# ilur98/DLMC-QUANT

Measured on NVIDIA B200. Metric: fakequant_fwd_bwd_hbm_gbps, higher is better.
Workload: dtype f32

## Files before the change

### dlmc_quant_b200/_lib.py

```python
import ctypes as C
import os

_HERE = os.path.dirname(os.path.abspath(__file__))
LIB_PATH = os.path.join(_HERE, "libdlmcq.so")

F32, BF16 = 0, 1
FORM_A1, FORM_AFFINE, FORM_ZP, FORM_SYM = 0, 1, 2, 3
STATS_PER_CHANNEL = 4
DIV_IEEE, DIV_CUDA_EAGER = 0, 1
SWEEP_CANDIDATES = 80
ROOTQ_STATE_FLOATS = 8
QGEMM_I8, QGEMM_E4M3 = 0, 1


class Layout(C.Structure):
    _fields_ = [("outer", C.c_int64), ("channels", C.c_int64), ("inner", C.c_int64), ("dtype", C.c_int32)]


class QParams(C.Structure):
    _fields_ = [("form", C.c_int32), ("lo", C.c_int32), ("hi", C.c_int32), ("g", C.c_float),
                ("scale", C.c_void_p), ("offset", C.c_void_p)]


class GroupItem(C.Structure):
# ... 36 lines not shown
                ("inner", C.c_int64), ("n_bits", C.c_int32), ("is_signed", C.c_int32), ("wpr", C.c_int32),
                ("row_floats", C.c_int32), ("staged", C.c_int32), ("pad", C.c_int32), ("smem_bytes", C.c_int64),
                ("ctas", C.c_int64)]


class BnqDesc(C.Structure):
    _fields_ = [("rows", C.c_int64), ("channels", C.c_int64), ("dtype", C.c_int32), ("flags", C.c_int32),
                ("eps", C.c_float), ("momentum", C.c_float)]


BNQ_TRAINING, BNQ_RELU, BNQ_RESIDUAL = 1, 2, 4


class DlmcqError(RuntimeError):
    pass


_lib = None

_P, _I, _L, _F, _D, _Z = C.c_void_p, C.c_int, C.c_int64, C.c_float, C.c_double, C.c_size_t
_LP, _QP = C.POINTER(Layout), C.POINTER(QParams)

SIGNATURES = {
    "dlmcq_version": (_I, []),
    "dlmcq_selftest_fastdiv": (_I, [C.c_uint64, _I, _I, _I, _P, _P]),
    "dlmcq_status_string": (C.c_char_p, [_I]),
    "dlmcq_last_cuda_error": (C.c_char_p, []),
    "dlmcq_workspace_bytes": (_Z, [_LP]),
    "dlmcq_fq_forward": (_I, [_P, _P, _P, _LP, _QP, _P]),
    "dlmcq_fq_backward": (_I, [_P, _P, _P, _P, _P, _LP, _QP, _P, _Z, _P]),
    "dlmcq_fq_partials_floats": (_Z, []),
    "dlmcq_fq_backward_partials": (_I, [_P, _P, _P, _LP, _QP, _P, _P]),
    "dlmcq_fq_finalize_many": (_I, [_P, _I, _P]),
    "dlmcq_dequantize": (_I, [_P, _P, _LP, _P, _P, _P]),
    "dlmcq_ste_value": (_I, [_P, _P, _L, _I, _I, _P]),
    "dlmcq_grad_scale_value": (_I, [_P, _P, _L, _F, _P]),
    "dlmcq_export_codes": (_I, [_P, _P, _LP, _QP, _I, _P]),
    "dlmcq_import_codes": (_I, [_P, _P, _LP, _QP, _I, _P]),
    "dlmcq_adaround_forward": (_I, [_P, _P, _P, _LP, _P, _I, _I, _I, _P]),
    "dlmcq_adaround_backward": (_I, [_P, _P, _P, _P, _P, _LP, _P, _I, _I, _P, _Z, _P]),
    "dlmcq_adaround_init_alpha": (_I, [_P, _P, _LP, _P, _P]),
    "dlmcq_rootq_act_prepare": (_I, [_P, _P, _D, _D, _I, _I, _I, _P, _P]),
    "dlmcq_rootq_act_forward": (_I, [_P, _P, _L, _I, _P, _P]),
    "dlmcq_rootq_act_backward": (_I, [_P, _P, _P, _P, _L, _I, _P, _P, _Z, _P]),
    "dlmcq_rootq_wt_prepare": (_I, [_P, _P, _P, _P, _P, _D, _D, _I, _I, _I, _P, _P]),
    "dlmcq_rootq_wt_forward": (_I, [_P, _P, _L, _I, _P, _P]),
    "dlmcq_rootq_wt_backward": (_I, [_P, _P, _P, _P, _L, _I, _P, _P, _Z, _P]),
    "dlmcq_rootq_prepare_many": (_I, [_P, _I, _P]),
    "dlmcq_rootq_wt_forward_grouped": (_I, [_P, _P, _I, _L, _I, _P]),
    "dlmcq_rootq_wt_backward_grouped": (_I, [_P, _P, _I, _L, _I, _P, _P]),
    "dlmcq_rootq_act_forward_grouped": (_I, [_P, _P, _I, _L, _I, _P]),
    "dlmcq_rootq_act_backward_grouped": (_I, [_P, _P, _I, _L, _I, _P, _P]),
    "dlmcq_obs_stats": (_I, [_P, _P, _LP, _I, _P, _Z, _P]),
    "dlmcq_obs_minmax_finalize": (_I, [_P, _P, _P, _L, _I, _I, _I, _P]),
    "dlmcq_obs_minmax_finalize_mode": (_I, [_P, _P, _P, _L, _I, _I, _I, _I, _P]),
    "dlmcq_obs_absmean_finalize": (_I, [_P, _P, _L, _D, _D, _D, _I, _P]),
    "dlmcq_obs_kth_state_bytes": (_Z, []),
    "dlmcq_obs_kth_begin": (_I, [_P, _L, _L, _P]),
    "dlmcq_obs_kth_hist": (_I, [_P, _L, _I, _I, _I, _P, _P]),
    "dlmcq_obs_kth_select": (_I, [_I, _P, _P]),
    "dlmcq_obs_kth_values": (_I, [_P, _P, _P]),
    "dlmcq_obs_kth_fast_workspace_bytes": (_Z, [_L]),
    "dlmcq_obs_kth_fast": (_I, [_P, _L, _I, _I, _L, _L, _P, _P, _P, _Z, _P]),
    "dlmcq_obs_kth_auto": (_I, [_P, _L, _I, _I, _L, _L, _P, _P, _P, _P, _Z, _P]),
    "dlmcq_obs_sweep_tensor_sse": (_I, [_P, _L, _I, _P, _I, _I, _P, _P, _Z, _P]),
    "dlmcq_obs_sweep_tensor_finalize": (_I, [_P, _P, _D, _I, _I, _P, _P, _P, _P]),
# ... 50 lines not shown
```

### dlmc_quant_b200/csrc/fq_kernels.cu

```cuda
#include "fq_rows.cuh"

namespace dlmcq {

constexpr int kUnroll = 4;

template <int FORM, typename T, int U = kUnroll, int MINB = 4, bool TILED = false>
__global__ void __launch_bounds__(kThreads, MINB)
fq_fwd_flat(const T* __restrict__ x, T* __restrict__ y, T* __restrict__ codes, int64_t n,
            const float* __restrict__ scale, const float* __restrict__ offset, float g, float lo, float hi) {
  using V = Vec<T>;
  using raw = typename V::raw;
  pdl_wait();
  pdl_trigger();
  const ChanParams p = make_params<FORM>(scale, offset, 0, g, lo, hi);
  const int64_t nvec = n / V::N;
  const int64_t stride = static_cast<int64_t>(gridDim.x) * blockDim.x;
  int64_t i = static_cast<int64_t>(blockIdx.x) * blockDim.x + threadIdx.x;
  const raw* xv = reinterpret_cast<const raw*>(x);
  raw* yv = reinterpret_cast<raw*>(y);
  raw* cv = reinterpret_cast<raw*>(codes);

  auto body = [&](const raw& r, int64_t idx) {
    float f[V::N], fy[V::N], fc[V::N];
    V::unpack(r, f);
    fq_vec<FORM, V::N>(f, p, lo, hi, fc, fy);
    if (y) st_stream(yv + idx, V::pack(fy));
    if (codes) st_stream(cv + idx, V::pack(fc));
  };
  if (TILED) {
    const int64_t tile_vecs = static_cast<int64_t>(U) * blockDim.x;
    const int64_t ntiles = nvec / tile_vecs;
    for (int64_t t = blockIdx.x; t < ntiles; t += gridDim.x) {
      const int64_t b = t * tile_vecs + threadIdx.x;
      raw r[U];
#pragma unroll
      for (int k = 0; k < U; ++k) r[k] = ld_stream(xv + b + k * blockDim.x);
#pragma unroll
      for (int k = 0; k < U; ++k) body(r[k], b + k * blockDim.x);
    }
    for (int64_t j = ntiles * tile_vecs + i; j < nvec; j += stride) body(ld_stream(xv + j), j);
  } else {
    for (; i + (U - 1) * stride < nvec; i += U * stride) {
      raw r[U];
#pragma unroll
      for (int k = 0; k < U; ++k) r[k] = ld_stream(xv + i + k * stride);
#pragma unroll
      for (int k = 0; k < U; ++k) body(r[k], i + k * stride);
    }
    for (; i < nvec; i += stride) body(ld_stream(xv + i), i);
  }
  if (blockIdx.x == 0) {
    const int64_t t = nvec * V::N + threadIdx.x;
    if (t < n) {
      float c, v;
      fq_elem<FORM>(to_f32<T>(x[t]), p, lo, hi, c, v);
      if (y) y[t] = from_f32<T>(v);
      if (codes) codes[t] = from_f32<T>(c);
    }
  }
}

template <int FORM, typename T>
__global__ void __launch_bounds__(kThreads)
fq_fwd_flat_unaligned(const T* __restrict__ x, T* __restrict__ y, T* __restrict__ codes, int64_t n,
                      const float* __restrict__ scale, const float* __restrict__ offset, float g, float lo, float hi) {
// ... 6 lines not shown
    if (codes) codes[i] = from_f32<T>(c);
  }
}

template <int FORM>
__device__ __forceinline__ void finalize_flat(float* partials, int nblocks, float g, float* dscale, float* doffset,
                                              float* smem) {
  double s = 0.0, o = 0.0;
  for (int b = threadIdx.x; b < nblocks; b += blockDim.x) {
    s += static_cast<double>(partials[2 * b]);
    o += static_cast<double>(partials[2 * b + 1]);
  }
  s = warp_sum(s);
  o = warp_sum(o);
  double* sm = reinterpret_cast<double*>(smem);
  const int lane = threadIdx.x & 31, warp = threadIdx.x >> 5, nwarp = blockDim.x >> 5;
  __syncthreads();
  if (lane == 0) { sm[warp] = s; sm[32 + warp] = o; }
  __syncthreads();
  if (threadIdx.x == 0) {
    double ts = 0.0, to = 0.0;
    for (int w = 0; w < nwarp; ++w) { ts += sm[w]; to += sm[32 + w]; }
    float r = static_cast<float>(ts);
    if (FORM == DLMCQ_FORM_AFFINE || FORM == DLMCQ_FORM_A1) r = r * g;
    dscale[0] = r;
    if (doffset) doffset[0] = static_cast<float>(to);
  }
}

template <int FORM, typename T, bool VECTOR, bool WANT_OFF, bool DEFER>
__global__ void __launch_bounds__(kThreads, 4)
fq_bwd_flat(const T* __restrict__ x, const T* __restrict__ dy, T* __restrict__ dx, int64_t n,
            const float* __restrict__ scale, const float* __restrict__ offset, float g, float lo, float hi,
            float* __restrict__ dscale, float* __restrict__ doffset, void* ws) {
  using V = Vec<T>;
  using raw = typename V::raw;
  __shared__ __align__(16) float smem[128];
  pdl_wait();
  pdl_trigger();
  const ChanParams p = make_params<FORM>(scale, offset, 0, g, lo, hi);
  float acc[2] = {0.f, 0.f};
  const int64_t stride = static_cast<int64_t>(gridDim.x) * blockDim.x;
  int64_t i = static_cast<int64_t>(blockIdx.x) * blockDim.x + threadIdx.x;
  if (VECTOR) {
    const int64_t nvec = n / V::N;
    const raw* xv = reinterpret_cast<const raw*>(x);
    const raw* gv = reinterpret_cast<const raw*>(dy);
    raw* ov = reinterpret_cast<raw*>(dx);
    auto body = [&](const raw& rx, const raw& rg, int64_t idx) {
      float fx[V::N], fg[V::N], fo[V::N];
      V::unpack(rx, fx);
      V::unpack(rg, fg);
      fq_vec_bwd<FORM, WANT_OFF, V::N>(fx, fg, p, lo, hi, fo, acc[0], acc[1]);
      st_stream(ov + idx, V::pack(fo));
    };
    const int64_t tile_vecs = static_cast<int64_t>(kUnroll) * blockDim.x;
    const int64_t ntiles = nvec / tile_vecs;
    for (int64_t t = blockIdx.x; t < ntiles; t += gridDim.x) {
      const int64_t b = t * tile_vecs + threadIdx.x;
      raw rx[kUnroll], rg[kUnroll];
#pragma unroll
      for (int k = 0; k < kUnroll; ++k) {
        rx[k] = ld_stream(xv + b + k * blockDim.x);
        rg[k] = ld_stream(gv + b + k * blockDim.x);
      }
#pragma unroll
      for (int k = 0; k < kUnroll; ++k) body(rx[k], rg[k], b + k * blockDim.x);
    }
    for (int64_t j = ntiles * tile_vecs + i; j < nvec; j += stride) body(ld_stream(xv + j), ld_stream(gv + j), j);
    if (blockIdx.x == 0) {
      const int64_t t = nvec * V::N + threadIdx.x;
      if (t < n) dx[t] = from_f32<T>(fq_elem_bwd<FORM, WANT_OFF>(to_f32<T>(x[t]), to_f32<T>(dy[t]), p, lo, hi, acc[0], acc[1]));
    }
  } else {
    for (; i < n; i += stride)
      dx[i] = from_f32<T>(fq_elem_bwd<FORM, WANT_OFF>(to_f32<T>(x[i]), to_f32<T>(dy[i]), p, lo, hi, acc[0], acc[1]));
  }
  block_sum<2>(acc, smem);
  if (DEFER) {
    float* out = static_cast<float*>(ws);
    if (threadIdx.x == 0) {
      if (blockIdx.x == 0) {
        out[0] = __int_as_float(static_cast<int>(gridDim.x));
        out[1] = (FORM == DLMCQ_FORM_AFFINE || FORM == DLMCQ_FORM_A1) ? g : 1.f;
      }
      out[2 + 2 * blockIdx.x] = acc[0];
      out[3 + 2 * blockIdx.x] = acc[1];
    }
    return;
  }
  float* partials = ws_partials(ws);
// ... 336 lines not shown
  }
}

__global__ void __launch_bounds__(128)
tiled_chan_finalize(const float* __restrict__ part, TileGeom gm, int64_t outer, float gmul, float* __restrict__ dscale) {
  __shared__ double sh[4];
  const int64_t ch = blockIdx.x;
  double s = 0.0;
  for (int64_t b = threadIdx.x; b < outer; b += blockDim.x) {
    const int64_t row = b * gm.channels + ch;
    const int64_t t0 = (row * gm.vpr) / kTileVecs, t1 = ((row + 1) * gm.vpr - 1) / kTileVecs;
    for (int64_t t = t0; t <= t1; ++t) {
      const int64_t row_first = (t * kTileVecs) / gm.vpr;
      s += static_cast<double>(part[t * kTileRows + (row - row_first)]);
    }
  }
  s = warp_sum(s);
  if ((threadIdx.x & 31) == 0) sh[threadIdx.x >> 5] = s;
  __syncthreads();
  if (threadIdx.x == 0) dscale[ch] = static_cast<float>((sh[0] + sh[1]) + (sh[2] + sh[3])) * gmul;
}

static inline int check_layout(const dlmcq_layout* l) {
  if (!l || l->outer < 1 || l->channels < 1 || l->inner < 0) return DLMCQ_EINVAL;
  if (l->dtype != DLMCQ_F32 && l->dtype != DLMCQ_BF16) return DLMCQ_EINVAL;
  return DLMCQ_OK;
}
static inline size_t elem_size(int dtype) { return dtype == DLMCQ_F32 ? 4 : 2; }
static inline bool elem_aligned(const void* p, int dtype) {
  return p == nullptr || (reinterpret_cast<uintptr_t>(p) % elem_size(dtype)) == 0;
}
static inline RowGeom make_geom(const dlmcq_layout* l) { return make_geom(l->outer, l->channels, l->inner); }

template <int FORM, typename T>
static int launch_fwd(const void* x, void* y, void* codes, const dlmcq_layout* l, const dlmcq_qparams* qp,
                      cudaStream_t st) {
  const int64_t n = l->outer * l->channels * l->inner;
  if (n == 0) return DLMCQ_OK;
  const float lo = static_cast<float>(qp->lo), hi = static_cast<float>(qp->hi);
  if (l->channels == 1) {
    if (aligned16(x) && aligned16(y) && aligned16(codes)) {
      const int64_t tiles = (n / Vec<T>::N + kThreads * kUnroll - 1) / (kThreads * kUnroll);
      auto kern = fq_fwd_flat<FORM, T, kUnroll, 4, true>;
      const int bps = 1024;
      cudaError_t e = launch_pdl(kern, dim3(stream_grid(tiles, bps)), dim3(kThreads), 0, st,
                                 static_cast<const T*>(x), static_cast<T*>(y), static_cast<T*>(codes), n, qp->scale,
                                 qp->offset, qp->g, lo, hi);
      if (e != cudaSuccess) return set_cuda_error(e);
    } else {
      const int64_t tiles = (n + kThreads - 1) / kThreads;
      fq_fwd_flat_unaligned<FORM, T><<<stream_grid(tiles, 8), kThreads, 0, st>>>(
          static_cast<const T*>(x), static_cast<T*>(y), static_cast<T*>(codes), n, qp->scale, qp->offset, qp->g, lo, hi);
    }
  } else if (tiled_ok<T>(l, x, y, codes)) {
    const TileGeom tg = make_tile_geom<T>(l);
    const int64_t tiles = (tg.nvec + kTileVecs - 1) / kTileVecs;
    if (tiles > 0x7fffffffLL) return DLMCQ_EUNSUPPORTED;
    fq_tiled_chan_kernel<FORM, T, false><<<static_cast<unsigned>(tiles), kThreads, 0, st>>>(
        static_cast<const T*>(x), nullptr, static_cast<T*>(y), static_cast<T*>(codes), tg, qp->scale, qp->offset,
        qp->g, lo, hi, nullptr);
  } else if (slab_ok<T>(l->outer, l->channels, l->inner, x, y, codes, nullptr)) {
    const SlabGeom sg = make_slab<T>(l->outer, l->channels, l->inner);
    fq_slab_kernel<FORM, T><<<static_cast<unsigned>(sg.groups) * sg.chunks, kThreads, 0, st>>>(
        static_cast<const T*>(x), static_cast<T*>(y), static_cast<T*>(codes), sg, qp->scale, qp->offset, qp->g, lo, hi);
  } else if (cmaj_ok(l->outer, l->channels, l->inner)) {
    const bool vec = cmaj_vec_ok<T>(l->inner, x, y, codes, nullptr);
    const CmajGeom cg = make_cmaj(l->outer, l->channels, l->inner, vec ? Vec<T>::N : 1);
    const int64_t blocks = (cg.channels * cg.chunks + kRowWarps - 1) / kRowWarps;
    if (blocks > 0x7fffffffLL) return DLMCQ_EUNSUPPORTED;
    auto kern = vec ? fq_cmaj_kernel<FORM, T, false, Vec<T>::N> : fq_cmaj_kernel<FORM, T, false, 1>;
    kern<<<static_cast<unsigned>(blocks), kRowWarps * 32, 0, st>>>(
        static_cast<const T*>(x), nullptr, static_cast<T*>(y), static_cast<T*>(codes), cg, qp->scale, qp->offset,
        qp->g, lo, hi, nullptr, nullptr, 0);
  } else {
    const RowGeom gm = make_geom(l);
    const int64_t items = gm.rows * gm.segs;
    const int64_t blocks = (items + kRowWarps - 1) / kRowWarps;
    if (blocks > 0x7fffffffLL) return DLMCQ_EUNSUPPORTED;
    fq_fwd_rows<FORM, T><<<static_cast<unsigned>(blocks), kRowWarps * 32, 0, st>>>(
        static_cast<const T*>(x), static_cast<T*>(y), static_cast<T*>(codes), gm, qp->scale, qp->offset, qp->g, lo, hi);
  }
  DLMCQ_LAUNCH_CHECK();
  return DLMCQ_OK;
}

template <int FORM, typename T>
static int launch_bwd(const void* x, const void* dy, void* dx, float* dscale, float* doffset, const dlmcq_layout* l,
                      const dlmcq_qparams* qp, void* ws, size_t ws_bytes, cudaStream_t st, bool defer = false) {
  const int64_t n = l->outer * l->channels * l->inner;
  const float lo = static_cast<float>(qp->lo), hi = static_cast<float>(qp->hi);
  if (!defer && ws_bytes < dlmcq_workspace_bytes(l)) return DLMCQ_EWORKSPACE;
  if (defer && l->channels != 1) return DLMCQ_EUNSUPPORTED;
  if (l->channels == 1) {
    const bool vec = aligned16(x) && aligned16(dy) && aligned16(dx);
    const int64_t per = vec ? Vec<T>::N : 1;
    int64_t tiles = (n / per + kThreads * kUnroll - 1) / (kThreads * kUnroll);
    int64_t cap = n < (int64_t(1) << 25) ? 888 : (n < (int64_t(1) << 27) ? 2048 : 4096);
    if (cap > kMaxPartialBlocks) cap = kMaxPartialBlocks;
    const int grid = static_cast<int>(tiles < 1 ? 1 : (tiles < cap ? tiles : cap));
    auto k = vec ? (doffset ? fq_bwd_flat<FORM, T, true, true, false> : fq_bwd_flat<FORM, T, true, false, false>)
                 : (doffset ? fq_bwd_flat<FORM, T, false, true, false> : fq_bwd_flat<FORM, T, false, false, false>);
    if (defer) k = vec ? fq_bwd_flat<FORM, T, true, false, true> : fq_bwd_flat<FORM, T, false, false, true>;
    cudaError_t e = launch_pdl(k, dim3(grid), dim3(kThreads), 0, st, static_cast<const T*>(x),
                               static_cast<const T*>(dy), static_cast<T*>(dx), n, qp->scale, qp->offset, qp->g, lo, hi,
                               dscale, doffset, ws);
    if (e != cudaSuccess) return set_cuda_error(e);
  } else if (doffset == nullptr && n > 0 && tiled_ok<T>(l, x, dy, dx)) {
    const TileGeom tg = make_tile_geom<T>(l);
    const int64_t tiles = (tg.nvec + kTileVecs - 1) / kTileVecs;
    if (tiles > 0x7fffffffLL) return DLMCQ_EUNSUPPORTED;
    fq_tiled_chan_kernel<FORM, T, true><<<static_cast<unsigned>(tiles), kThreads, 0, st>>>(
        static_cast<const T*>(x), static_cast<const T*>(dy), static_cast<T*>(dx), nullptr, tg, qp->scale, qp->offset,
        qp->g, lo, hi, ws_partials(ws));
    DLMCQ_LAUNCH_CHECK();
    const float gmul = (FORM == DLMCQ_FORM_AFFINE || FORM == DLMCQ_FORM_A1) ? qp->g : 1.f;
    tiled_chan_finalize<<<static_cast<unsigned>(l->channels), 128, 0, st>>>(ws_partials(ws), tg, l->outer, gmul, dscale);
  } else if (cmaj_ok(l->outer, l->channels, l->inner) && doffset == nullptr && n > 0) {
    const bool vec = cmaj_vec_ok<T>(l->inner, x, dy, dx, nullptr);
    const CmajGeom cg = make_cmaj(l->outer, l->channels, l->inner, vec ? Vec<T>::N : 1);
    const int64_t blocks = (cg.channels * cg.chunks + kRowWarps - 1) / kRowWarps;
    if (blocks > 0x7fffffffLL) return DLMCQ_EUNSUPPORTED;
    const int direct = cg.chunks == 1 ? 1 : 0;
    auto kern = vec ? fq_cmaj_kernel<FORM, T, true, Vec<T>::N> : fq_cmaj_kernel<FORM, T, true, 1>;
    kern<<<static_cast<unsigned>(blocks), kRowWarps * 32, 0, st>>>(
        static_cast<const T*>(x), static_cast<const T*>(dy), static_cast<T*>(dx), nullptr, cg, qp->scale, qp->offset,
        qp->g, lo, hi, dscale, ws_partials(ws), direct);
    if (!direct) {
      DLMCQ_LAUNCH_CHECK();
      const float gmul = (FORM == DLMCQ_FORM_AFFINE || FORM == DLMCQ_FORM_A1) ? qp->g : 1.f;
      chan_finalize<1><<<static_cast<unsigned>(cg.channels), 128, 0, st>>>(ws_partials(ws), cg.chunks, cg.chunks, 0,
                                                                           gmul, dscale, nullptr);
    }
  } else {
    const RowGeom gm = make_geom(l);
    const int64_t items = gm.rows * gm.segs;
    const int64_t blocks = (items + kRowWarps - 1) / kRowWarps;
    if (blocks > 0x7fffffffLL) return DLMCQ_EUNSUPPORTED;
    const int direct = (l->outer == 1 && gm.segs == 1) ? 1 : 0;
    if (n == 0) return DLMCQ_OK;
// ... 7 lines not shown
          ws_partials(ws), l->outer * gm.segs, gm.segs, gm.channels * gm.segs, gmul, dscale, doffset);
    }
  }
  DLMCQ_LAUNCH_CHECK();
  return DLMCQ_OK;
}

template <typename T>
static int dispatch_fwd(const void* x, void* y, void* codes, const dlmcq_layout* l, const dlmcq_qparams* qp,
                        cudaStream_t st) {
  switch (qp->form) {
    case DLMCQ_FORM_A1: return launch_fwd<DLMCQ_FORM_A1, T>(x, y, codes, l, qp, st);
    case DLMCQ_FORM_AFFINE: return launch_fwd<DLMCQ_FORM_AFFINE, T>(x, y, codes, l, qp, st);
    case DLMCQ_FORM_ZP: return launch_fwd<DLMCQ_FORM_ZP, T>(x, y, codes, l, qp, st);
    case DLMCQ_FORM_SYM: return launch_fwd<DLMCQ_FORM_SYM, T>(x, y, codes, l, qp, st);
  }
  return DLMCQ_EINVAL;
}
template <typename T>
static int dispatch_bwd(const void* x, const void* dy, void* dx, float* ds, float* doff, const dlmcq_layout* l,
                        const dlmcq_qparams* qp, void* ws, size_t wsb, cudaStream_t st, bool defer = false) {
  switch (qp->form) {
    case DLMCQ_FORM_A1: return launch_bwd<DLMCQ_FORM_A1, T>(x, dy, dx, ds, doff, l, qp, ws, wsb, st, defer);
    case DLMCQ_FORM_AFFINE: return launch_bwd<DLMCQ_FORM_AFFINE, T>(x, dy, dx, ds, doff, l, qp, ws, wsb, st, defer);
    case DLMCQ_FORM_ZP: return launch_bwd<DLMCQ_FORM_ZP, T>(x, dy, dx, ds, doff, l, qp, ws, wsb, st, defer);
    case DLMCQ_FORM_SYM: return launch_bwd<DLMCQ_FORM_SYM, T>(x, dy, dx, ds, doff, l, qp, ws, wsb, st, defer);
  }
  return DLMCQ_EINVAL;
}

__global__ void __launch_bounds__(kThreads)
finalize_many_kernel(const dlmcq_finalize_item* __restrict__ items, int n_items) {
  __shared__ double sm[2][kThreads / 32];
  const dlmcq_finalize_item it = items[blockIdx.x];
  const float* p = it.partials;
  const int nblocks = __float_as_int(p[0]);
  const float gmul = p[1];
  double s = 0.0, o = 0.0;
  for (int b = threadIdx.x; b < nblocks; b += blockDim.x) {
    s += static_cast<double>(p[2 + 2 * b]);
    o += static_cast<double>(p[3 + 2 * b]);
  }
  s = warp_sum(s);
  o = warp_sum(o);
  const int lane = threadIdx.x & 31, warp = threadIdx.x >> 5;
  if (lane == 0) { sm[0][warp] = s; sm[1][warp] = o; }
  __syncthreads();
  if (threadIdx.x == 0) {
    double ts = 0.0, to = 0.0;
    for (int w = 0; w < kThreads / 32; ++w) { ts += sm[0][w]; to += sm[1][w]; }
    it.dscale[0] = static_cast<float>(ts) * gmul;
    (void)to;
  }
}

}

using namespace dlmcq;

extern "C" size_t dlmcq_workspace_bytes(const dlmcq_layout* l) {
  size_t bytes = kWsHeaderBytes + static_cast<size_t>(kMaxPartialBlocks) * 96 * sizeof(float);
  if (l && l->outer >= 1 && l->channels >= 1 && l->inner >= 0) {
    const RowGeom gm = make_geom(l->outer, l->channels, l->inner);
    const size_t rows_bytes = static_cast<size_t>(gm.rows * gm.segs) * 4 * sizeof(float);
    if (kWsHeaderBytes + rows_bytes > bytes) bytes = kWsHeaderBytes + rows_bytes;
    const size_t tiles = static_cast<size_t>(l->outer * l->channels * l->inner) / (kTileVecs * 4) + 1;
// ... 33 lines not shown
                                const float* offset, void* stream) {
  if (int e = check_layout(layout)) return e;
  if (!codes || !y || !scale) return DLMCQ_EINVAL;
  const int64_t n = layout->outer * layout->channels * layout->inner;
  if (n == 0) return DLMCQ_OK;
  cudaStream_t st = static_cast<cudaStream_t>(stream);
  const int grid = stream_grid((n + kThreads - 1) / kThreads, 8);
  if (layout->dtype == DLMCQ_F32)
    dequant_kernel<float><<<grid, kThreads, 0, st>>>(static_cast<const float*>(codes), static_cast<float*>(y), n,
                                                     layout->channels, layout->inner, scale, offset);
  else
    dequant_kernel<__nv_bfloat16><<<grid, kThreads, 0, st>>>(static_cast<const __nv_bfloat16*>(codes),
                                                             static_cast<__nv_bfloat16*>(y), n, layout->channels,
                                                             layout->inner, scale, offset);
  DLMCQ_LAUNCH_CHECK();
  return DLMCQ_OK;
}

extern "C" size_t dlmcq_fq_partials_floats(void) { return 2 + 2 * static_cast<size_t>(kMaxPartialBlocks); }

extern "C" int dlmcq_fq_backward_partials(const void* x, const void* dy, void* dx, const dlmcq_layout* layout,
                                          const dlmcq_qparams* qp, float* partials, void* stream) {
  if (int e = check_layout(layout)) return e;
  if (layout->channels != 1) return DLMCQ_EUNSUPPORTED;
  if (!qp || !qp->scale || !partials || !x || !dy || !dx) return DLMCQ_EINVAL;
  if (!elem_aligned(x, layout->dtype) || !elem_aligned(dy, layout->dtype) || !elem_aligned(dx, layout->dtype))
    return DLMCQ_EALIGN;
  cudaStream_t st = static_cast<cudaStream_t>(stream);
  return layout->dtype == DLMCQ_F32
             ? dispatch_bwd<float>(x, dy, dx, nullptr, nullptr, layout, qp, partials, 0, st, true)
             : dispatch_bwd<__nv_bfloat16>(x, dy, dx, nullptr, nullptr, layout, qp, partials, 0, st, true);
}

extern "C" int dlmcq_fq_finalize_many(const dlmcq_finalize_item* items, int n_items, void* stream) {
  if (!items || n_items < 0) return DLMCQ_EINVAL;
  if (n_items == 0) return DLMCQ_OK;
  finalize_many_kernel<<<n_items, kThreads, 0, static_cast<cudaStream_t>(stream)>>>(items, n_items);
  DLMCQ_LAUNCH_CHECK();
  return DLMCQ_OK;
}
```

### dlmc_quant_b200/csrc/grouped_kernels.cu

```cuda
#include "fq_rows.cuh"

namespace dlmcq {

__device__ __forceinline__ int find_item(const int64_t* __restrict__ prefix, int n_items, int64_t unit) {
  int lo = 0, hi = n_items;
  while (hi - lo > 1) {
    const int mid = (lo + hi) >> 1;
    if (__ldg(prefix + mid) <= unit) lo = mid; else hi = mid;
  }
  return lo;
}

template <int FORM>
__device__ __forceinline__ ChanParams item_params(const dlmcq_group_item& it, int64_t ch) {
  return make_params<FORM>(it.scale, it.offset, ch, it.g, static_cast<float>(it.lo), static_cast<float>(it.hi));
}

template <typename T>
__global__ void __launch_bounds__(kRowWarps * 32)
grouped_fwd_kernel(const dlmcq_group_item* __restrict__ items, const int64_t* __restrict__ prefix, int n_items,
                   int64_t total_units) {
  const int lane = threadIdx.x & 31;
  const int64_t unit = static_cast<int64_t>(blockIdx.x) * kRowWarps + (threadIdx.x >> 5);
  if (unit >= total_units) return;
  const int k = find_item(prefix, n_items, unit);
  const dlmcq_group_item it = items[k];
  const int64_t local = unit - __ldg(prefix + k);
  const int64_t segs = (it.inner + DLMCQ_GROUP_SEG - 1) / DLMCQ_GROUP_SEG;
  const int64_t row = local / segs, seg = local - row * segs;
  const int64_t beg = seg * DLMCQ_GROUP_SEG;
  const int64_t len = (it.inner - beg) < DLMCQ_GROUP_SEG ? (it.inner - beg) : DLMCQ_GROUP_SEG;
  const T* xr = static_cast<const T*>(it.x) + row * it.inner + beg;
  T* yr = static_cast<T*>(it.y) + row * it.inner + beg;
  const float lo = static_cast<float>(it.lo), hi = static_cast<float>(it.hi);
  switch (it.form) {
    case DLMCQ_FORM_A1: fwd_row_segment<DLMCQ_FORM_A1, T>(xr, yr, nullptr, len, item_params<DLMCQ_FORM_A1>(it, row), lo, hi, lane); break;
    case DLMCQ_FORM_AFFINE: fwd_row_segment<DLMCQ_FORM_AFFINE, T>(xr, yr, nullptr, len, item_params<DLMCQ_FORM_AFFINE>(it, row), lo, hi, lane); break;
    case DLMCQ_FORM_ZP: fwd_row_segment<DLMCQ_FORM_ZP, T>(xr, yr, nullptr, len, item_params<DLMCQ_FORM_ZP>(it, row), lo, hi, lane); break;
    default: fwd_row_segment<DLMCQ_FORM_SYM, T>(xr, yr, nullptr, len, item_params<DLMCQ_FORM_SYM>(it, row), lo, hi, lane); break;
  }
}

template <typename T>
__global__ void __launch_bounds__(kRowWarps * 32)
grouped_bwd_kernel(const dlmcq_group_item* __restrict__ items, const int64_t* __restrict__ prefix, int n_items,
                   int64_t total_units, float* __restrict__ partials) {
  const int lane = threadIdx.x & 31;
  const int64_t unit = static_cast<int64_t>(blockIdx.x) * kRowWarps + (threadIdx.x >> 5);
  if (unit >= total_units) return;
  const int k = find_item(prefix, n_items, unit);
  const dlmcq_group_item it = items[k];
  const int64_t local = unit - __ldg(prefix + k);
  const int64_t segs = (it.inner + DLMCQ_GROUP_SEG - 1) / DLMCQ_GROUP_SEG;
  const int64_t row = local / segs, seg = local - row * segs;
  const int64_t beg = seg * DLMCQ_GROUP_SEG;
  const int64_t len = (it.inner - beg) < DLMCQ_GROUP_SEG ? (it.inner - beg) : DLMCQ_GROUP_SEG;
  const int64_t base = row * it.inner + beg;
  const T* xr = static_cast<const T*>(it.x) + base;
  const T* gr = static_cast<const T*>(it.dy) + base;
  T* dr = static_cast<T*>(it.y) + base;
  const float lo = static_cast<float>(it.lo), hi = static_cast<float>(it.hi);
  float as = 0.f, ao = 0.f;
  switch (it.form) {
    case DLMCQ_FORM_A1: bwd_row_segment<DLMCQ_FORM_A1, T>(xr, gr, dr, len, item_params<DLMCQ_FORM_A1>(it, row), lo, hi, lane, as, ao); break;
    case DLMCQ_FORM_AFFINE: bwd_row_segment<DLMCQ_FORM_AFFINE, T>(xr, gr, dr, len, item_params<DLMCQ_FORM_AFFINE>(it, row), lo, hi, lane, as, ao); break;
    case DLMCQ_FORM_ZP: bwd_row_segment<DLMCQ_FORM_ZP, T>(xr, gr, dr, len, item_params<DLMCQ_FORM_ZP>(it, row), lo, hi, lane, as, ao); break;
    default: bwd_row_segment<DLMCQ_FORM_SYM, T>(xr, gr, dr, len, item_params<DLMCQ_FORM_SYM>(it, row), lo, hi, lane, as, ao); break;
  }
  if (lane == 0) partials[unit] = as;
}

__global__ void __launch_bounds__(kRowWarps * 32)
grouped_finalize_kernel(const dlmcq_group_item* __restrict__ items, const int64_t* __restrict__ prefix,
                        const int64_t* __restrict__ chan_prefix, int n_items, int64_t total_channels,
                        const float* __restrict__ partials) {
  const int lane = threadIdx.x & 31;
  const int64_t gch = static_cast<int64_t>(blockIdx.x) * kRowWarps + (threadIdx.x >> 5);
  if (gch >= total_channels) return;
  const int k = find_item(chan_prefix, n_items, gch);
  const dlmcq_group_item it = items[k];
  const int64_t ch = gch - __ldg(chan_prefix + k);
  const int64_t segs = (it.inner + DLMCQ_GROUP_SEG - 1) / DLMCQ_GROUP_SEG;
  const float* p = partials + __ldg(prefix + k) + ch * segs;
  double s = 0.0;
  for (int64_t j = lane; j < segs; j += 32) s += static_cast<double>(p[j]);
  s = warp_sum(s);
  if (lane == 0) {
    float r = static_cast<float>(s);
    if (it.form == DLMCQ_FORM_AFFINE || it.form == DLMCQ_FORM_A1) r = r * it.g;
    it.dscale[ch] = r;
  }
}

}

using namespace dlmcq;

extern "C" int dlmcq_fq_forward_grouped(const dlmcq_group_item* items, const int64_t* unit_prefix, int n_items,
                                        int64_t total_units, int dtype, void* stream) {
  if (!items || !unit_prefix || n_items < 1 || total_units < 0) return DLMCQ_EINVAL;
  if (total_units == 0) return DLMCQ_OK;
  const int64_t blocks = (total_units + kRowWarps - 1) / kRowWarps;
  if (blocks > 0x7fffffffLL) return DLMCQ_EUNSUPPORTED;
  cudaStream_t st = static_cast<cudaStream_t>(stream);
  if (dtype == DLMCQ_F32)
    grouped_fwd_kernel<float><<<static_cast<unsigned>(blocks), kRowWarps * 32, 0, st>>>(items, unit_prefix, n_items, total_units);
  else if (dtype == DLMCQ_BF16)
    grouped_fwd_kernel<__nv_bfloat16><<<static_cast<unsigned>(blocks), kRowWarps * 32, 0, st>>>(items, unit_prefix, n_items, total_units);
  else
    return DLMCQ_EINVAL;
  DLMCQ_LAUNCH_CHECK();
  return DLMCQ_OK;
}

extern "C" int dlmcq_fq_backward_grouped(const dlmcq_group_item* items, const int64_t* unit_prefix,
                                         const int64_t* chan_prefix, int n_items, int64_t total_units,
                                         int64_t total_channels, int dtype, float* partials, void* stream) {
  if (!items || !unit_prefix || !chan_prefix || !partials || n_items < 1 || total_units < 0) return DLMCQ_EINVAL;
  if (total_units == 0) return DLMCQ_OK;
  const int64_t blocks = (total_units + kRowWarps - 1) / kRowWarps;
  const int64_t fblocks = (total_channels + kRowWarps - 1) / kRowWarps;
  if (blocks > 0x7fffffffLL || fblocks > 0x7fffffffLL) return DLMCQ_EUNSUPPORTED;
  cudaStream_t st = static_cast<cudaStream_t>(stream);
  if (dtype == DLMCQ_F32)
    grouped_bwd_kernel<float><<<static_cast<unsigned>(blocks), kRowWarps * 32, 0, st>>>(items, unit_prefix, n_items, total_units, partials);
  else if (dtype == DLMCQ_BF16)
    grouped_bwd_kernel<__nv_bfloat16><<<static_cast<unsigned>(blocks), kRowWarps * 32, 0, st>>>(items, unit_prefix, n_items, total_units, partials);
  else
    return DLMCQ_EINVAL;
  DLMCQ_LAUNCH_CHECK();
  grouped_finalize_kernel<<<static_cast<unsigned>(fblocks), kRowWarps * 32, 0, st>>>(items, unit_prefix, chan_prefix, n_items, total_channels, partials);
  DLMCQ_LAUNCH_CHECK();
  return DLMCQ_OK;
}
```

### include/dlmcq.h

```cpp
#ifndef DLMCQ_H_
#define DLMCQ_H_

#include <stddef.h>
#include <stdint.h>

#ifdef __cplusplus
extern "C" {
#endif

#define DLMCQ_VERSION 100

typedef enum {
  DLMCQ_OK = 0,
  DLMCQ_EINVAL = -1,
  DLMCQ_EALIGN = -2,
  DLMCQ_EWORKSPACE = -3,
  DLMCQ_ECUDA = -4,
  DLMCQ_EUNSUPPORTED = -5
} dlmcq_status;

typedef enum { DLMCQ_F32 = 0, DLMCQ_BF16 = 1 } dlmcq_dtype;

typedef enum {
  DLMCQ_FORM_A1 = 0,
// ... 10 lines not shown
} dlmcq_layout;

typedef struct {
  int32_t form;
  int32_t lo, hi;
  float g;
  const float* scale;
  const float* offset;
} dlmcq_qparams;

int dlmcq_version(void);
int dlmcq_selftest_fastdiv(uint64_t seed, int blocks, int per_thread, int narrow,
                           unsigned long long* mismatches_dev, void* stream);
const char* dlmcq_status_string(int status);
const char* dlmcq_last_cuda_error(void);

size_t dlmcq_workspace_bytes(const dlmcq_layout* layout);

int dlmcq_fq_forward(const void* x, void* y, void* codes, const dlmcq_layout* layout,
                     const dlmcq_qparams* qp, void* stream);

int dlmcq_fq_backward(const void* x, const void* dy, void* dx, float* dscale, float* doffset,
                      const dlmcq_layout* layout, const dlmcq_qparams* qp,
                      void* workspace, size_t workspace_bytes, void* stream);

typedef struct {
  const float* partials;
  float* dscale;
} dlmcq_finalize_item;
size_t dlmcq_fq_partials_floats(void);
int dlmcq_fq_backward_partials(const void* x, const void* dy, void* dx, const dlmcq_layout* layout,
                               const dlmcq_qparams* qp, float* partials, void* stream);
int dlmcq_fq_finalize_many(const dlmcq_finalize_item* items, int n_items, void* stream);

int dlmcq_ste_value(const void* x, void* y, int64_t numel, int dtype, int mode, void* stream);
int dlmcq_grad_scale_value(const float* s, float* out, int64_t numel, float g, void* stream);

int dlmcq_dequantize(const void* codes, void* y, const dlmcq_layout* layout,
                     const float* scale, const float* offset, void* stream);

int dlmcq_export_codes(const void* x, void* codes_out, const dlmcq_layout* layout, const dlmcq_qparams* qp,
                       int pack4, void* stream);
int dlmcq_import_codes(const void* codes, void* y, const dlmcq_layout* layout, const dlmcq_qparams* qp,
                       int pack4, void* stream);

int dlmcq_adaround_forward(const void* w, const void* alpha, void* y, const dlmcq_layout* layout,
                           const float* scale, int lo, int hi, int soft, void* stream);
int dlmcq_adaround_backward(const void* w, const void* alpha, const void* dy, void* dalpha,
                            float* dscale, const dlmcq_layout* layout, const float* scale,
                            int lo, int hi, void* workspace, size_t workspace_bytes, void* stream);
int dlmcq_adaround_init_alpha(const void* w, void* alpha, const dlmcq_layout* layout,
                              const float* scale, void* stream);

#define DLMCQ_ROOTQ_STATE_FLOATS 8

int dlmcq_rootq_act_prepare(const float* in_scale, float* run_scale, double momentum, double g,
                            int lo, int hi, int training, float* state, void* stream);
int dlmcq_rootq_act_forward(const void* x, void* y, int64_t numel, int dtype,
                            const float* state, void* stream);
int dlmcq_rootq_act_backward(const void* x, const void* dy, void* dx, float* d_in_scale,
                             int64_t numel, int dtype, const float* state,
                             void* workspace, size_t workspace_bytes, void* stream);
int dlmcq_rootq_wt_prepare(const float* upper, const float* lower, const float* alpha,
                           float* run_upper, float* run_lower, double momentum, double g,
                           int lo, int hi, int training, float* state, void* stream);
int dlmcq_rootq_wt_forward(const void* w, void* y, int64_t numel, int dtype,
// ... 177 lines not shown
```

Measured before the change: 6293.

## Prefetch first tile before PDL wait when captured kernels touch disjoint memory

During CUDA graph capture, each flat fake-quant launch records the byte ranges it reads and writes, and checks them against the previous captured node. When the ranges do not overlap, the kernel loads its first tile and quant params before pdl_wait, so its memory reads overlap the tail of the previous kernel. Finalize and grouped kernels are also moved to PDL launches with wait/trigger. The cost is host-side bookkeeping with a mutex and extra registers for the hoisted tile, and correctness depends on the alias check covering every dependency.

```diff
diff --git a/dlmc_quant_b200/_lib.py b/dlmc_quant_b200/_lib.py
--- a/dlmc_quant_b200/_lib.py
+++ b/dlmc_quant_b200/_lib.py
@@ -92,6 +92,7 @@
     "dlmcq_fq_partials_floats": (_Z, []),
     "dlmcq_fq_backward_partials": (_I, [_P, _P, _P, _LP, _QP, _P, _P]),
     "dlmcq_fq_finalize_many": (_I, [_P, _I, _P]),
+    "dlmcq_capture_overlap_count": (_I, []),
     "dlmcq_dequantize": (_I, [_P, _P, _LP, _P, _P, _P]),
     "dlmcq_ste_value": (_I, [_P, _P, _L, _I, _I, _P]),
     "dlmcq_grad_scale_value": (_I, [_P, _P, _L, _F, _P]),
diff --git a/dlmc_quant_b200/csrc/fq_kernels.cu b/dlmc_quant_b200/csrc/fq_kernels.cu
--- a/dlmc_quant_b200/csrc/fq_kernels.cu
+++ b/dlmc_quant_b200/csrc/fq_kernels.cu
@@ -1,3 +1,5 @@
+#include <mutex>
+
 #include "fq_rows.cuh"
 
 namespace dlmcq {
@@ -7,16 +9,30 @@
 template <int FORM, typename T, int U = kUnroll, int MINB = 4, bool TILED = false>
 __global__ void __launch_bounds__(kThreads, MINB)
 fq_fwd_flat(const T* __restrict__ x, T* __restrict__ y, T* __restrict__ codes, int64_t n,
-            const float* __restrict__ scale, const float* __restrict__ offset, float g, float lo, float hi) {
+            const float* __restrict__ scale, const float* __restrict__ offset, float g, float lo, float hi,
+            int independent) {
   using V = Vec<T>;
   using raw = typename V::raw;
+  const int64_t nvec = n / V::N;
+  const raw* xv = reinterpret_cast<const raw*>(x);
+  const int64_t tile_vecs = static_cast<int64_t>(U) * blockDim.x;
+  const int64_t ntiles = nvec / tile_vecs;
+  ChanParams p;
+  raw r0[U];
+  const bool hoist = TILED && independent && blockIdx.x < ntiles;
+  if (TILED && independent) {
+    p = make_params<FORM>(scale, offset, 0, g, lo, hi);
+    if (hoist) {
+      const int64_t b = static_cast<int64_t>(blockIdx.x) * tile_vecs + threadIdx.x;
+#pragma unroll
+      for (int k = 0; k < U; ++k) r0[k] = ld_stream(xv + b + k * blockDim.x);
+    }
+  }
   pdl_wait();
   pdl_trigger();
-  const ChanParams p = make_params<FORM>(scale, offset, 0, g, lo, hi);
-  const int64_t nvec = n / V::N;
+  if (!(TILED && independent)) p = make_params<FORM>(scale, offset, 0, g, lo, hi);
   const int64_t stride = static_cast<int64_t>(gridDim.x) * blockDim.x;
   int64_t i = static_cast<int64_t>(blockIdx.x) * blockDim.x + threadIdx.x;
-  const raw* xv = reinterpret_cast<const raw*>(x);
   raw* yv = reinterpret_cast<raw*>(y);
   raw* cv = reinterpret_cast<raw*>(codes);
 
@@ -28,9 +44,14 @@
     if (codes) st_stream(cv + idx, V::pack(fc));
   };
   if (TILED) {
-    const int64_t tile_vecs = static_cast<int64_t>(U) * blockDim.x;
-    const int64_t ntiles = nvec / tile_vecs;
-    for (int64_t t = blockIdx.x; t < ntiles; t += gridDim.x) {
+    int64_t t = blockIdx.x;
+    if (hoist) {
+      const int64_t b = t * tile_vecs + threadIdx.x;
+#pragma unroll
+      for (int k = 0; k < U; ++k) body(r0[k], b + k * blockDim.x);
+      t += gridDim.x;
+    }
+    for (; t < ntiles; t += gridDim.x) {
       const int64_t b = t * tile_vecs + threadIdx.x;
       raw r[U];
 #pragma unroll
@@ -103,20 +124,36 @@
 __global__ void __launch_bounds__(kThreads, 4)
 fq_bwd_flat(const T* __restrict__ x, const T* __restrict__ dy, T* __restrict__ dx, int64_t n,
             const float* __restrict__ scale, const float* __restrict__ offset, float g, float lo, float hi,
-            float* __restrict__ dscale, float* __restrict__ doffset, void* ws) {
+            float* __restrict__ dscale, float* __restrict__ doffset, void* ws, int independent) {
   using V = Vec<T>;
   using raw = typename V::raw;
   __shared__ __align__(16) float smem[128];
+  const int64_t nvec = n / V::N;
+  const raw* xv = reinterpret_cast<const raw*>(x);
+  const raw* gv = reinterpret_cast<const raw*>(dy);
+  const int64_t tile_vecs = static_cast<int64_t>(kUnroll) * blockDim.x;
+  const int64_t ntiles = nvec / tile_vecs;
+  ChanParams p;
+  raw rx0[kUnroll], rg0[kUnroll];
+  const bool hoist = VECTOR && independent && blockIdx.x < ntiles;
+  if (VECTOR && independent) {
+    p = make_params<FORM>(scale, offset, 0, g, lo, hi);
+    if (hoist) {
+      const int64_t b = static_cast<int64_t>(blockIdx.x) * tile_vecs + threadIdx.x;
+#pragma unroll
+      for (int k = 0; k < kUnroll; ++k) {
+        rx0[k] = ld_stream(xv + b + k * blockDim.x);
+        rg0[k] = ld_stream(gv + b + k * blockDim.x);
+      }
+    }
+  }
   pdl_wait();
   pdl_trigger();
-  const ChanParams p = make_params<FORM>(scale, offset, 0, g, lo, hi);
+  if (!(VECTOR && independent)) p = make_params<FORM>(scale, offset, 0, g, lo, hi);
   float acc[2] = {0.f, 0.f};
   const int64_t stride = static_cast<int64_t>(gridDim.x) * blockDim.x;
   int64_t i = static_cast<int64_t>(blockIdx.x) * blockDim.x + threadIdx.x;
   if (VECTOR) {
-    const int64_t nvec = n / V::N;
-    const raw* xv = reinterpret_cast<const raw*>(x);
-    const raw* gv = reinterpret_cast<const raw*>(dy);
     raw* ov = reinterpret_cast<raw*>(dx);
     auto body = [&](const raw& rx, const raw& rg, int64_t idx) {
       float fx[V::N], fg[V::N], fo[V::N];
@@ -125,9 +162,14 @@
       fq_vec_bwd<FORM, WANT_OFF, V::N>(fx, fg, p, lo, hi, fo, acc[0], acc[1]);
       st_stream(ov + idx, V::pack(fo));
     };
-    const int64_t tile_vecs = static_cast<int64_t>(kUnroll) * blockDim.x;
-    const int64_t ntiles = nvec / tile_vecs;
-    for (int64_t t = blockIdx.x; t < ntiles; t += gridDim.x) {
+    int64_t t = blockIdx.x;
+    if (hoist) {
+      const int64_t b = t * tile_vecs + threadIdx.x;
+#pragma unroll
+      for (int k = 0; k < kUnroll; ++k) body(rx0[k], rg0[k], b + k * blockDim.x);
+      t += gridDim.x;
+    }
+    for (; t < ntiles; t += gridDim.x) {
       const int64_t b = t * tile_vecs + threadIdx.x;
       raw rx[kUnroll], rg[kUnroll];
 #pragma unroll
@@ -530,6 +572,73 @@
 }
 static inline RowGeom make_geom(const dlmcq_layout* l) { return make_geom(l->outer, l->channels, l->inner); }
 
+struct ByteRange {
+  uintptr_t beg, end;
+};
+struct FlatAccess {
+  ByteRange rd[5], wr[6];
+  int nrd = 0, nwr = 0;
+  void read(const void* p, size_t bytes) {
+    if (p && bytes) rd[nrd++] = {reinterpret_cast<uintptr_t>(p), reinterpret_cast<uintptr_t>(p) + bytes};
+  }
+  void write(const void* p, size_t bytes) {
+    if (p && bytes) wr[nwr++] = {reinterpret_cast<uintptr_t>(p), reinterpret_cast<uintptr_t>(p) + bytes};
+  }
+};
+struct CaptureLast {
+  unsigned long long id;
+  cudaGraphNode_t node;
+  FlatAccess acc;
+};
+constexpr int kCaptureSlots = 16;
+static std::mutex g_capture_mu;
+static CaptureLast g_capture[kCaptureSlots];
+static int g_capture_next = 0;
+static thread_local int g_overlap_count = 0;
+
+static bool capture_tip(cudaStream_t st, unsigned long long* id, cudaGraphNode_t* node) {
+  cudaStreamCaptureStatus status = cudaStreamCaptureStatusNone;
+  const cudaGraphNode_t* deps = nullptr;
+  size_t ndeps = 0;
+  if (cudaStreamGetCaptureInfo(st, &status, id, nullptr, &deps, &ndeps) != cudaSuccess) {
+    (void)cudaGetLastError();
+    return false;
+  }
+  if (status != cudaStreamCaptureStatusActive || ndeps != 1 || deps[0] == nullptr) return false;
+  *node = deps[0];
+  return true;
+}
+
+static int capture_check(cudaStream_t st, const FlatAccess& a) {
+  unsigned long long id = 0;
+  cudaGraphNode_t node = nullptr;
+  if (!pdl_enabled() || !capture_tip(st, &id, &node)) return 0;
+  std::lock_guard<std::mutex> lock(g_capture_mu);
+  for (const CaptureLast& c : g_capture) {
+    if (c.node != node || c.id != id) continue;
+    for (int r = 0; r < a.nrd; ++r)
+      for (int w = 0; w < c.acc.nwr; ++w)
+        if (a.rd[r].beg < c.acc.wr[w].end && c.acc.wr[w].beg < a.rd[r].end) return 0;
+    return 1;
+  }
+  return 0;
+}
+
+static void capture_record(cudaStream_t st, const FlatAccess& a, int independent) {
+  unsigned long long id = 0;
+  cudaGraphNode_t node = nullptr;
+  if (!pdl_enabled() || !capture_tip(st, &id, &node)) return;
+  if (independent) ++g_overlap_count;
+  std::lock_guard<std::mutex> lock(g_capture_mu);
+  CaptureLast* slot = nullptr;
+  for (CaptureLast& c : g_capture)
+    if (c.node != nullptr && c.id == id) slot = &c;
+  if (!slot) slot = &g_capture[g_capture_next++ % kCaptureSlots];
+  slot->id = id;
+  slot->node = node;
+  slot->acc = a;
+}
+
 template <int FORM, typename T>
 static int launch_fwd(const void* x, void* y, void* codes, const dlmcq_layout* l, const dlmcq_qparams* qp,
                       cudaStream_t st) {
@@ -541,10 +650,19 @@
       const int64_t tiles = (n / Vec<T>::N + kThreads * kUnroll - 1) / (kThreads * kUnroll);
       auto kern = fq_fwd_flat<FORM, T, kUnroll, 4, true>;
       const int bps = 1024;
+      const size_t bytes = static_cast<size_t>(n) * sizeof(T);
+      FlatAccess acc;
+      acc.read(x, bytes);
+      acc.read(qp->scale, sizeof(float));
+      acc.read(qp->offset, sizeof(float));
+      acc.write(y, bytes);
+      acc.write(codes, bytes);
+      const int independent = capture_check(st, acc);
       cudaError_t e = launch_pdl(kern, dim3(stream_grid(tiles, bps)), dim3(kThreads), 0, st,
                                  static_cast<const T*>(x), static_cast<T*>(y), static_cast<T*>(codes), n, qp->scale,
-                                 qp->offset, qp->g, lo, hi);
+                                 qp->offset, qp->g, lo, hi, independent);
       if (e != cudaSuccess) return set_cuda_error(e);
+      capture_record(st, acc, independent);
     } else {
       const int64_t tiles = (n + kThreads - 1) / kThreads;
       fq_fwd_flat_unaligned<FORM, T><<<stream_grid(tiles, 8), kThreads, 0, st>>>(
@@ -599,10 +717,25 @@
     auto k = vec ? (doffset ? fq_bwd_flat<FORM, T, true, true, false> : fq_bwd_flat<FORM, T, true, false, false>)
                  : (doffset ? fq_bwd_flat<FORM, T, false, true, false> : fq_bwd_flat<FORM, T, false, false, false>);
     if (defer) k = vec ? fq_bwd_flat<FORM, T, true, false, true> : fq_bwd_flat<FORM, T, false, false, true>;
+    FlatAccess acc;
+    if (vec) {
+      const size_t bytes = static_cast<size_t>(n) * sizeof(T);
+      acc.read(x, bytes);
+      acc.read(dy, bytes);
+      acc.read(qp->scale, sizeof(float));
+      acc.read(qp->offset, sizeof(float));
+      if (!defer) acc.read(ws, ws_bytes);
+      acc.write(dx, bytes);
+      acc.write(dscale, sizeof(float));
+      acc.write(doffset, sizeof(float));
+      acc.write(ws, defer ? (2 + 2 * static_cast<size_t>(grid)) * sizeof(float) : ws_bytes);
+    }
+    const int independent = vec ? capture_check(st, acc) : 0;
     cudaError_t e = launch_pdl(k, dim3(grid), dim3(kThreads), 0, st, static_cast<const T*>(x),
                                static_cast<const T*>(dy), static_cast<T*>(dx), n, qp->scale, qp->offset, qp->g, lo, hi,
-                               dscale, doffset, ws);
+                               dscale, doffset, ws, independent);
     if (e != cudaSuccess) return set_cuda_error(e);
+    if (vec) capture_record(st, acc, independent);
   } else if (doffset == nullptr && n > 0 && tiled_ok<T>(l, x, dy, dx)) {
     const TileGeom tg = make_tile_geom<T>(l);
     const int64_t tiles = (tg.nvec + kTileVecs - 1) / kTileVecs;
@@ -676,6 +809,8 @@
 __global__ void __launch_bounds__(kThreads)
 finalize_many_kernel(const dlmcq_finalize_item* __restrict__ items, int n_items) {
   __shared__ double sm[2][kThreads / 32];
+  pdl_wait();
+  pdl_trigger();
   const dlmcq_finalize_item it = items[blockIdx.x];
   const float* p = it.partials;
   const int nblocks = __float_as_int(p[0]);
@@ -775,10 +910,17 @@
              : dispatch_bwd<__nv_bfloat16>(x, dy, dx, nullptr, nullptr, layout, qp, partials, 0, st, true);
 }
 
+extern "C" int dlmcq_capture_overlap_count(void) {
+  const int n = g_overlap_count;
+  g_overlap_count = 0;
+  return n;
+}
+
 extern "C" int dlmcq_fq_finalize_many(const dlmcq_finalize_item* items, int n_items, void* stream) {
   if (!items || n_items < 0) return DLMCQ_EINVAL;
   if (n_items == 0) return DLMCQ_OK;
-  finalize_many_kernel<<<n_items, kThreads, 0, static_cast<cudaStream_t>(stream)>>>(items, n_items);
-  DLMCQ_LAUNCH_CHECK();
+  cudaError_t e = launch_pdl(finalize_many_kernel, dim3(n_items), dim3(kThreads), 0, static_cast<cudaStream_t>(stream),
+                             items, n_items);
+  if (e != cudaSuccess) return set_cuda_error(e);
   return DLMCQ_OK;
 }
diff --git a/dlmc_quant_b200/csrc/grouped_kernels.cu b/dlmc_quant_b200/csrc/grouped_kernels.cu
--- a/dlmc_quant_b200/csrc/grouped_kernels.cu
+++ b/dlmc_quant_b200/csrc/grouped_kernels.cu
@@ -20,6 +20,8 @@
 __global__ void __launch_bounds__(kRowWarps * 32)
 grouped_fwd_kernel(const dlmcq_group_item* __restrict__ items, const int64_t* __restrict__ prefix, int n_items,
                    int64_t total_units) {
+  pdl_wait();
+  pdl_trigger();
   const int lane = threadIdx.x & 31;
   const int64_t unit = static_cast<int64_t>(blockIdx.x) * kRowWarps + (threadIdx.x >> 5);
   if (unit >= total_units) return;
@@ -45,6 +47,8 @@
 __global__ void __launch_bounds__(kRowWarps * 32)
 grouped_bwd_kernel(const dlmcq_group_item* __restrict__ items, const int64_t* __restrict__ prefix, int n_items,
                    int64_t total_units, float* __restrict__ partials) {
+  pdl_wait();
+  pdl_trigger();
   const int lane = threadIdx.x & 31;
   const int64_t unit = static_cast<int64_t>(blockIdx.x) * kRowWarps + (threadIdx.x >> 5);
   if (unit >= total_units) return;
@@ -74,6 +78,8 @@
 grouped_finalize_kernel(const dlmcq_group_item* __restrict__ items, const int64_t* __restrict__ prefix,
                         const int64_t* __restrict__ chan_prefix, int n_items, int64_t total_channels,
                         const float* __restrict__ partials) {
+  pdl_wait();
+  pdl_trigger();
   const int lane = threadIdx.x & 31;
   const int64_t gch = static_cast<int64_t>(blockIdx.x) * kRowWarps + (threadIdx.x >> 5);
   if (gch >= total_channels) return;
@@ -103,13 +109,11 @@
   const int64_t blocks = (total_units + kRowWarps - 1) / kRowWarps;
   if (blocks > 0x7fffffffLL) return DLMCQ_EUNSUPPORTED;
   cudaStream_t st = static_cast<cudaStream_t>(stream);
-  if (dtype == DLMCQ_F32)
-    grouped_fwd_kernel<float><<<static_cast<unsigned>(blocks), kRowWarps * 32, 0, st>>>(items, unit_prefix, n_items, total_units);
-  else if (dtype == DLMCQ_BF16)
-    grouped_fwd_kernel<__nv_bfloat16><<<static_cast<unsigned>(blocks), kRowWarps * 32, 0, st>>>(items, unit_prefix, n_items, total_units);
-  else
-    return DLMCQ_EINVAL;
-  DLMCQ_LAUNCH_CHECK();
+  if (dtype != DLMCQ_F32 && dtype != DLMCQ_BF16) return DLMCQ_EINVAL;
+  cudaError_t e = launch_pdl(dtype == DLMCQ_F32 ? grouped_fwd_kernel<float> : grouped_fwd_kernel<__nv_bfloat16>,
+                             dim3(static_cast<unsigned>(blocks)), dim3(kRowWarps * 32), 0, st, items, unit_prefix,
+                             n_items, total_units);
+  if (e != cudaSuccess) return set_cuda_error(e);
   return DLMCQ_OK;
 }
 
@@ -122,14 +126,13 @@
   const int64_t fblocks = (total_channels + kRowWarps - 1) / kRowWarps;
   if (blocks > 0x7fffffffLL || fblocks > 0x7fffffffLL) return DLMCQ_EUNSUPPORTED;
   cudaStream_t st = static_cast<cudaStream_t>(stream);
-  if (dtype == DLMCQ_F32)
-    grouped_bwd_kernel<float><<<static_cast<unsigned>(blocks), kRowWarps * 32, 0, st>>>(items, unit_prefix, n_items, total_units, partials);
-  else if (dtype == DLMCQ_BF16)
-    grouped_bwd_kernel<__nv_bfloat16><<<static_cast<unsigned>(blocks), kRowWarps * 32, 0, st>>>(items, unit_prefix, n_items, total_units, partials);
-  else
-    return DLMCQ_EINVAL;
-  DLMCQ_LAUNCH_CHECK();
-  grouped_finalize_kernel<<<static_cast<unsigned>(fblocks), kRowWarps * 32, 0, st>>>(items, unit_prefix, chan_prefix, n_items, total_channels, partials);
-  DLMCQ_LAUNCH_CHECK();
+  if (dtype != DLMCQ_F32 && dtype != DLMCQ_BF16) return DLMCQ_EINVAL;
+  cudaError_t e = launch_pdl(dtype == DLMCQ_F32 ? grouped_bwd_kernel<float> : grouped_bwd_kernel<__nv_bfloat16>,
+                             dim3(static_cast<unsigned>(blocks)), dim3(kRowWarps * 32), 0, st, items, unit_prefix,
+                             n_items, total_units, partials);
+  if (e != cudaSuccess) return set_cuda_error(e);
+  e = launch_pdl(grouped_finalize_kernel, dim3(static_cast<unsigned>(fblocks)), dim3(kRowWarps * 32), 0, st, items,
+                 unit_prefix, chan_prefix, n_items, total_channels, partials);
+  if (e != cudaSuccess) return set_cuda_error(e);
   return DLMCQ_OK;
 }
diff --git a/include/dlmcq.h b/include/dlmcq.h
--- a/include/dlmcq.h
+++ b/include/dlmcq.h
@@ -66,6 +66,8 @@
 int dlmcq_fq_backward_partials(const void* x, const void* dy, void* dx, const dlmcq_layout* layout,
                                const dlmcq_qparams* qp, float* partials, void* stream);
 int dlmcq_fq_finalize_many(const dlmcq_finalize_item* items, int n_items, void* stream);
+
+int dlmcq_capture_overlap_count(void);
 
 int dlmcq_ste_value(const void* x, void* y, int64_t numel, int dtype, int mode, void* stream);
 int dlmcq_grad_scale_value(const float* s, float* out, int64_t numel, float g, void* stream);
diff --git a/profiles/capture_gaps.py b/profiles/capture_gaps.py
--- /dev/null
+++ b/profiles/capture_gaps.py
@@ -0,0 +1,64 @@
+import argparse
+import json
+import os
+import statistics
+import sys
+
+ROOT = os.path.dirname(os.path.dirname(os.path.abspath(__file__)))
+if ROOT not in sys.path:
+    sys.path.insert(0, ROOT)
+
+
+def main():
+    ap = argparse.ArgumentParser()
+    ap.add_argument("--batch", type=int, default=128)
+    ap.add_argument("--steps", type=int, default=3)
+    ap.add_argument("--out", default=None)
+    args = ap.parse_args()
+    import torch
+    from torch.profiler import ProfilerActivity, profile
+
+    import bench
+    wl = bench.Workload(args.batch, torch.device("cuda"), 2333)
+    wl.capture()
+    for _ in range(3):
+        wl.g_fwd.replay(); wl.g_bwd.replay(); wl.g_wt.replay()
+    torch.cuda.synchronize()
+    with profile(activities=[ProfilerActivity.CUDA]) as prof:
+        for _ in range(args.steps):
+            wl.g_fwd.replay(); wl.g_bwd.replay(); wl.g_wt.replay()
+        torch.cuda.synchronize()
+    kernels = sorted((e for e in prof.events() if e.device_type == torch.autograd.DeviceType.CUDA
+                      and e.name not in ("Memcpy", "Memset")), key=lambda e: e.time_range.start)
+    per_step = wl.launches_per_step
+    if len(kernels) < per_step * args.steps:
+        raise SystemExit(f"expected {per_step * args.steps} kernels in the trace, found {len(kernels)}")
+    step = kernels[-per_step:]
+    rows, gaps, adv = [], {"fwd": [], "bwd": [], "other": []}, {"fwd": [], "bwd": [], "other": []}
+    for a, b in zip(step, step[1:]):
+        gap = b.time_range.start - a.time_range.end
+        kind = ("fwd" if "fq_fwd_flat" in a.name and "fq_fwd_flat" in b.name else
+                "bwd" if "fq_bwd_flat" in a.name and "fq_bwd_flat" in b.name else "other")
+        advance = b.time_range.end - a.time_range.end
+        gaps[kind].append(gap)
+        adv[kind].append(advance)
+        rows.append({"prev": a.name.split("(")[0][:60], "next": b.name.split("(")[0][:60], "gap_us": round(gap, 2),
+                     "advance_us": round(advance, 2),
+                     "prev_us": round(a.time_range.end - a.time_range.start, 2)})
+    span = step[-1].time_range.end - step[0].time_range.start
+    busy = sum(k.time_range.end - k.time_range.start for k in step)
+    summary = {"batch": args.batch, "kernels_per_step": per_step,
+               "gpu": torch.cuda.get_device_name(), "step_span_us": round(span, 1),
+               "kernel_time_us": round(busy, 1), "span_minus_kernel_time_us": round(span - busy, 1)}
+    for kind, v in gaps.items():
+        if v:
+            summary[kind] = {"boundaries": len(v), "gap_sum_us": round(sum(v), 1),
+                             "gap_median_us": round(statistics.median(v), 2), "advance_sum_us": round(sum(adv[kind]), 1)}
+    print(json.dumps(summary), flush=True)
+    if args.out:
+        with open(args.out, "w") as f:
+            json.dump({"summary": summary, "boundaries": rows}, f, indent=1)
+
+
+if __name__ == "__main__":
+    main()
```

Measured after the change: 6568, median of 6. +4.4%, better.
